# caofff/GL-ABC-MCMC

Hardware: NVIDIA B200
Metric: abc_mcmc_chain_steps_per_sec (higher is better)
Workload: dtype f32

## Files before the change

### gl-abc-mcmc_b200/csrc/philox.cuh

```cuda
#pragma once
#include <cstdint>
#include <cuda_runtime.h>

namespace glabc {

constexpr uint32_t kPhiloxM0 = 0xD2511F53u;
constexpr uint32_t kPhiloxM1 = 0xCD9E8D57u;
constexpr uint32_t kPhiloxW0 = 0x9E3779B9u;
constexpr uint32_t kPhiloxW1 = 0xBB67AE85u;

constexpr uint32_t kSlotStep = 1u;
constexpr uint32_t kSlotNormal = 2u;
constexpr uint32_t kSlotU64 = 0x80000000u;

struct RoundKeys {
    uint32_t k[10][2];
};

__host__ __device__ inline RoundKeys expand_key(uint2 key)
{
    RoundKeys rk;
    for (int r = 0; r < 10; ++r) {
        rk.k[r][0] = key.x + static_cast<uint32_t>(r) * kPhiloxW0;
        rk.k[r][1] = key.y + static_cast<uint32_t>(r) * kPhiloxW1;
    }
    return rk;
}

__device__ __forceinline__ uint4 philox4x32_10(uint4 c, const RoundKeys& rk)
{
#pragma unroll
    for (int r = 0; r < 10; ++r) {
        const uint64_t p0 = static_cast<uint64_t>(kPhiloxM0) * c.x;
        const uint64_t p1 = static_cast<uint64_t>(kPhiloxM1) * c.z;
        c = make_uint4(static_cast<uint32_t>(p1 >> 32) ^ c.y ^ rk.k[r][0], static_cast<uint32_t>(p1),
                       static_cast<uint32_t>(p0 >> 32) ^ c.w ^ rk.k[r][1], static_cast<uint32_t>(p0));
    }
    return c;
}

struct Stream {
    uint32_t chain_lo, chain_hi;
    __device__ __forceinline__ uint4 block(const RoundKeys& rk, uint32_t blk, uint32_t slot) const
    {
        return philox4x32_10(make_uint4(chain_lo, chain_hi, blk, slot), rk);
    }
};

__device__ __forceinline__ float u24(uint32_t w) { return __uint2float_rn(w >> 8) * 0x1p-24f; }

__device__ __forceinline__ float lg2_approx(float x)
{
    float r;
    asm("lg2.approx.ftz.f32 %0, %1;" : "=f"(r) : "f"(x));
    return r;
}

__device__ __forceinline__ float log_approx(float x) { return 0.69314718055994531f * lg2_approx(x); }

__device__ __forceinline__ void box_muller(uint32_t w0, uint32_t w1, float& n0, float& n1)
{
    const float u1 = fmaf(__uint2float_rn(w0 & 0xFFFFFF00u), 0x1p-32f, 0x1p-25f);
    const float r2 = -1.3862943611198906f * lg2_approx(u1);
    float r;
    asm("sqrt.approx.ftz.f32 %0, %1;" : "=f"(r) : "f"(r2));
    const float a = __uint2float_rn(w1 & 0xFFFFF000u) * (6.28318530717958647692f * 0x1p-32f);
    n0 = r * __cosf(a);
    n1 = r * __sinf(a);
}

__device__ __forceinline__ uint32_t step_block_ub(const uint4& w) { return __byte_perm(w.x, w.z, 0x0400); }
__device__ __forceinline__ uint32_t step_block_ua(const uint4& w) { return (w.y & 0xFFFu) | ((w.w << 12) & 0xFFF000u); }

}
```

### gl-abc-mcmc_b200/csrc/sampler_common.cuh

```cuda
#pragma once
#include <cstdint>
#include <cuda_runtime.h>

#include "../../include/glabc.h"
#include "model.cuh"
#include "philox.cuh"

namespace glabc {

struct RunParams {
    int32_t n_chains;
    uint32_t first_step;
    uint32_t last_step;
    uint32_t chain_lo0, chain_hi0;
    RoundKeys rk;
    float gf;
    uint32_t gf_thr_hi;
    int32_t gf_all_global;
    int32_t write_row0;
    int64_t trace_rows, trace_chains, trace_chain_off, trace_row_base;
    float* theta;
    float* y;
    float* aux;
    float* trace;
    float* stats;
    const float* tape32;
    const double* tape64;
    float* debug;
    float* tape_dump;
    double* tape64_dump;
    int32_t n_candidates;
    int32_t trace_layout;
    double* state64;
    const float* tape_grad0;
    float* tape_grad0_dump;
    double* debug64;
};

__device__ __forceinline__ Stream chain_stream(const RunParams& r, int32_t chain)
{
    const uint64_t gid = (static_cast<uint64_t>(r.chain_hi0) << 32 | r.chain_lo0) + static_cast<uint64_t>(chain);
    return Stream{static_cast<uint32_t>(gid), static_cast<uint32_t>(gid >> 32)};
}

template <int D>
struct VecOf { using type = float; };
template <> struct VecOf<2> { using type = float2; };
template <> struct VecOf<4> { using type = float4; };

template <int D>
__device__ __forceinline__ void store_row(float* dst, const float (&v)[D])
{
    if constexpr (D == 2) {
        *reinterpret_cast<float2*>(dst) = make_float2(v[0], v[1]);
    } else if constexpr (D == 4) {
        *reinterpret_cast<float4*>(dst) = make_float4(v[0], v[1], v[2], v[3]);
    } else {
#pragma unroll
        for (int k = 0; k < D; ++k) dst[k] = v[k];
    }
}

template <int D>
struct TimeMajorWriter {
    float* next;
    bool active;
    __device__ __forceinline__ TimeMajorWriter(const RunParams& r, int32_t chain, bool act, float*)
        : active(act)
    {
        const int64_t first_row = static_cast<int64_t>(r.first_step) - (r.write_row0 ? 1 : 0) - r.trace_row_base;
        next = r.trace + (first_row * r.trace_chains + r.trace_chain_off + chain) * D;
    }
    __device__ __forceinline__ void put(const RunParams& r, uint32_t, const float (&v)[D])
    {
        if (active) store_row<D>(next, v);
        next += r.trace_chains * D;
    }
    __device__ __forceinline__ void maybe_flush(const RunParams&, uint32_t) {}
    __device__ __forceinline__ void finish(const RunParams&) {}
    static constexpr int smem_floats_per_warp = 0;
};

template <int D>
struct ChainMajorWriter {
    static constexpr int kPitch = 33;
    static constexpr int kPlane = 32 * kPitch + (D > 1 ? 32 / D : 0);
    static constexpr int smem_floats_per_warp = D * kPlane;
    float* tile;
    float* out;
    int64_t chain_stride;
    uint32_t row0;
    int32_t count;
    int32_t lane;
    int32_t chains_in_warp;

    __device__ __forceinline__ ChainMajorWriter(const RunParams& r, int32_t, bool, float* smem_warp)
        : tile(smem_warp), chain_stride(r.trace_rows * D), row0(0), count(0), lane(threadIdx.x & 31)
    {
        const int32_t chain0 = blockIdx.x * blockDim.x + (threadIdx.x & ~31u);
        out = r.trace + (r.trace_chain_off + chain0) * chain_stride;
        chains_in_warp = min(32, r.n_chains - chain0);
    }

    __device__ __forceinline__ void put(const RunParams& r, uint32_t row, const float (&v)[D])
    {
        if (count == 0) row0 = row;
#pragma unroll
        for (int k = 0; k < D; ++k) tile[k * kPlane + count * kPitch + lane] = v[k];
        ++count;
    }

    __device__ __forceinline__ void maybe_flush(const RunParams& r, uint32_t row)
    {
        if (((row + 1u) & 31u) == 0u) flush(r);
    }

    __device__ __forceinline__ void flush(const RunParams& r)
    {
        __syncwarp();
        const int32_t n = count * D;
        const int64_t off = (static_cast<int64_t>(row0) - r.trace_row_base) * D;
        for (int32_t c = 0; c < chains_in_warp; ++c) {
            float* dst = out + c * chain_stride + off;
            for (int32_t e = lane; e < n; e += 32) {
                const int32_t s = e / D, k = e - s * D;
                dst[e] = tile[k * kPlane + s * kPitch + c];
            }
        }
        __syncwarp();
        count = 0;
    }

    __device__ __forceinline__ void finish(const RunParams& r)
    {
        if (count > 0) flush(r);
    }
};

template <int D>
struct ChainMajorVecWriter {
    using V = typename VecOf<D>::type;
    static constexpr int kPitch = 33;
    static constexpr int smem_floats_per_warp = 32 * kPitch * D;
    V* tile;
    V* out;
    int64_t chain_stride;
    uint32_t row0;
    int32_t count, lane, chains_in_warp;

    __device__ __forceinline__ ChainMajorVecWriter(const RunParams& r, int32_t, bool, float* smem_warp)
        : tile(reinterpret_cast<V*>(smem_warp)), chain_stride(r.trace_rows), row0(0), count(0), lane(threadIdx.x & 31)
    {
        const int32_t chain0 = blockIdx.x * blockDim.x + (threadIdx.x & ~31u);
        out = reinterpret_cast<V*>(r.trace) + (r.trace_chain_off + chain0) * chain_stride;
        chains_in_warp = min(32, r.n_chains - chain0);
    }

    __device__ __forceinline__ void put(const RunParams&, uint32_t row, const float (&v)[D])
    {
        if (count == 0) row0 = row;
        V x;
        if constexpr (D == 1) x = v[0];
        else if constexpr (D == 2) x = make_float2(v[0], v[1]);
        else x = make_float4(v[0], v[1], v[2], v[3]);
        tile[count * kPitch + lane] = x;
        ++count;
    }

    __device__ __forceinline__ void maybe_flush(const RunParams& r, uint32_t row)
    {
        if (((row + 1u) & 31u) == 0u) flush(r);
    }

    __device__ __forceinline__ void flush(const RunParams& r)
    {
        __syncwarp();
        V* dst = out + (static_cast<int64_t>(row0) - r.trace_row_base) + lane;
        const V* src = tile + lane * kPitch;
        if (count == 32 && chains_in_warp == 32) {
#pragma unroll 8
            for (int32_t c = 0; c < 32; ++c) dst[c * chain_stride] = src[c];
        } else {
            for (int32_t c = 0; c < chains_in_warp; ++c)
                if (lane < count) dst[c * chain_stride] = src[c];
        }
        __syncwarp();
        count = 0;
    }

    __device__ __forceinline__ void finish(const RunParams& r)
    {
        if (count > 0) flush(r);
    }
};

template <int D>
struct EventWriter {
    float* ev;
    uint32_t n;
    uint32_t cap;
    float last[D];
    bool active;
    static constexpr int smem_floats_per_warp = 0;
    __device__ __forceinline__ EventWriter(const RunParams& r, int32_t chain, bool act, float*)
        : ev(r.trace + (r.trace_chain_off + chain) * r.trace_rows * (1 + D)), n(1u), cap(static_cast<uint32_t>(r.trace_rows)), active(act)
    {
#pragma unroll
        for (int k = 0; k < D; ++k) last[k] = __int_as_float(0x7fc00000);
    }
    __device__ __forceinline__ void put(const RunParams&, uint32_t row, const float (&v)[D])
    {
        bool moved = false;
#pragma unroll
        for (int k = 0; k < D; ++k) moved |= !(v[k] == last[k]);
        if (moved) {
            if (active && n < cap) {
                float* e = ev + static_cast<int64_t>(n) * (1 + D);
                e[0] = __uint_as_float(row);
#pragma unroll
                for (int k = 0; k < D; ++k) e[1 + k] = v[k];
            }
            ++n;
#pragma unroll
            for (int k = 0; k < D; ++k) last[k] = v[k];
        }
    }
    __device__ __forceinline__ void maybe_flush(const RunParams&, uint32_t) {}
    __device__ __forceinline__ void finish(const RunParams&)
    {
        if (active) ev[0] = __uint_as_float(n - 1u);
    }
};

struct NoTraceWriter {
    __device__ __forceinline__ NoTraceWriter(const RunParams&, int32_t, bool, float*) {}
    template <int D>
    __device__ __forceinline__ void put(const RunParams&, uint32_t, const float (&)[D]) {}
    __device__ __forceinline__ void maybe_flush(const RunParams&, uint32_t) {}
    __device__ __forceinline__ void finish(const RunParams&) {}
    static constexpr int smem_floats_per_warp = 0;
};

template <int D, int LAYOUT> struct WriterFor;
template <int D> struct WriterFor<D, GLABC_TRACE_NONE> { using type = NoTraceWriter; };
template <int D> struct WriterFor<D, GLABC_TRACE_TIME_MAJOR> { using type = TimeMajorWriter<D>; };
template <int D> struct WriterFor<D, GLABC_TRACE_CHAIN_MAJOR> { using type = ChainMajorVecWriter<D>; };
template <> struct WriterFor<3, GLABC_TRACE_CHAIN_MAJOR> { using type = ChainMajorWriter<3>; };
template <int D> struct WriterFor<D, GLABC_TRACE_EVENTS> { using type = EventWriter<D>; };

template <int D>
struct ChainStats {
    static constexpr int kTri = D * (D + 1) / 2;
    uint32_t n_global, acc_local, acc_global;
    float f_global, f_acc, f_acc_global;
    float sum[D], sumsq[D], gram[kTri];

    __device__ __forceinline__ ChainStats()
        : n_global(0), acc_local(0), acc_global(0), f_global(0.0f), f_acc(0.0f), f_acc_global(0.0f)
    {
#pragma unroll
        for (int i = 0; i < D; ++i) sum[i] = sumsq[i] = 0.0f;
#pragma unroll
        for (int i = 0; i < kTri; ++i) gram[i] = 0.0f;
    }

    __device__ __forceinline__ void update(bool is_global, bool moved, const float (&theta_new)[D],
                                           const float (&theta_prev)[D])
    {
        n_global += is_global;
        acc_global += (moved && is_global);
        acc_local += (moved && !is_global);
        float dl[D];
#pragma unroll
        for (int i = 0; i < D; ++i) {
            sum[i] += theta_new[i];
            sumsq[i] = fmaf(theta_new[i], theta_new[i], sumsq[i]);
            dl[i] = theta_new[i] - theta_prev[i];
        }
        int t = 0;
#pragma unroll
        for (int i = 0; i < D; ++i)
#pragma unroll
            for (int j = i; j < D; ++j, ++t) gram[t] = fmaf(dl[i], dl[j], gram[t]);
    }

    __device__ __forceinline__ void update_masked(float glob, float moved, const float (&theta_new)[D],
                                                  const float (&theta_prev)[D])
    {
        f_global += glob;
        f_acc += moved;
        f_acc_global = fmaf(moved, glob, f_acc_global);
        float dl[D];
#pragma unroll
        for (int i = 0; i < D; ++i) {
            sum[i] += theta_new[i];
            sumsq[i] = fmaf(theta_new[i], theta_new[i], sumsq[i]);
            dl[i] = theta_new[i] - theta_prev[i];
        }
        int t = 0;
#pragma unroll
        for (int i = 0; i < D; ++i)
#pragma unroll
            for (int j = i; j < D; ++j, ++t) gram[t] = fmaf(dl[i], dl[j], gram[t]);
    }

    __device__ __forceinline__ void store(float* st, uint32_t n_steps) const
    {
        st[GLABC_STAT_STEPS] += static_cast<float>(n_steps);
        st[GLABC_STAT_GLOBAL_STEPS] += static_cast<float>(n_global) + f_global;
        st[GLABC_STAT_ACC_LOCAL] += static_cast<float>(acc_local) + (f_acc - f_acc_global);
        st[GLABC_STAT_ACC_GLOBAL] += static_cast<float>(acc_global) + f_acc_global;
#pragma unroll
        for (int i = 0; i < D; ++i) {
            st[GLABC_STAT_SUM + i] += sum[i];
            st[GLABC_STAT_SUM + D + i] += sumsq[i];
        }
#pragma unroll
        for (int i = 0; i < kTri; ++i) st[GLABC_STAT_SUM + 2 * D + i] += gram[i];
    }
};

}
```

### gl-abc-mcmc_b200/csrc/step_global.cuh

```cuda
#pragma once
#include "launch.cuh"
#include "sampler_common.cuh"

namespace glabc {

struct GlobalConsts {
    ModelConsts model;
    GaussConsts lp;
    GaussConsts gp;
};

template <int D>
struct StepInputs {
    bool is_global;
    float keep;
    float glob;
    float cand[D];
    float noise[D];
    float lq_p;
    float log_w;
    float raw[2 * D + 2];
};

template <int D, bool STRICT, bool KEEP_RAW>
__device__ __forceinline__ StepInputs<D> make_inputs(const GlobalConsts& K, bool is_global, float u_b, float u_a,
                                                    const float (&eps_p)[D], const float (&eps_s)[D])
{
    StepInputs<D> in;
    in.is_global = is_global;
    in.keep = is_global ? 0.0f : 1.0f;
    in.glob = 1.0f - in.keep;
    if constexpr (STRICT) {
        float th_g[D], th_l[D];
        in.lq_p = gauss_forward<D, true>(K.gp, eps_p, th_g);
        (void)gauss_forward<D, true>(K.lp, eps_p, th_l);
#pragma unroll
        for (int k = 0; k < D; ++k) {
            in.cand[k] = is_global ? th_g[k] : th_l[k];
            in.noise[k] = __fadd_rn(K.model.noise_loc[k], __fmul_rn(K.model.noise_scale[k], eps_s[k]));
        }
        in.log_w = logf(u_a);
    } else {
        float q = 0.0f;
#pragma unroll
        for (int k = 0; k < D; ++k) {
            const float cg = fmaf(K.gp.scale[k], eps_p[k], K.gp.loc[k]);
            const float cl = fmaf(K.lp.scale[k], eps_p[k], K.lp.loc[k]);
            in.cand[k] = is_global ? cg : cl;
            in.noise[k] = fmaf(K.model.noise_scale[k], eps_s[k], K.model.noise_loc[k]);
            q = fmaf(eps_p[k], eps_p[k], q);
        }
        in.lq_p = fmaf(-0.5f, q, K.gp.c_fast);
        in.log_w = fmaf(in.glob, in.lq_p, log_approx(u_a));
    }
    if constexpr (KEEP_RAW) {
        in.raw[0] = u_b;
#pragma unroll
        for (int k = 0; k < D; ++k) {
            in.raw[1 + k] = eps_p[k];
            in.raw[1 + D + k] = eps_s[k];
        }
        in.raw[1 + 2 * D] = u_a;
    }
    return in;
}

template <int D, bool STRICT>
__device__ __forceinline__ StepInputs<D> inputs_from_tape(const GlobalConsts& K, const RunParams& r,
                                                         uint32_t step_in_launch, int32_t chain)
{
    constexpr int kSlots = GLABC_TAPE_GLOBAL_SLOTS(D, D);
    const float* t = r.tape32 + (static_cast<int64_t>(step_in_launch) * kSlots) * r.n_chains + chain;
    float eps_p[D], eps_s[D];
    const float u_b = __ldg(t);
#pragma unroll
    for (int k = 0; k < D; ++k) eps_p[k] = __ldg(t + static_cast<int64_t>(1 + k) * r.n_chains);
#pragma unroll
    for (int k = 0; k < D; ++k) eps_s[k] = __ldg(t + static_cast<int64_t>(1 + D + k) * r.n_chains);
    const float u_a = __ldg(t + static_cast<int64_t>(1 + 2 * D) * r.n_chains);
    return make_inputs<D, STRICT, false>(K, u_b < r.gf, u_b, u_a, eps_p, eps_s);
}

template <int D, bool STRICT, bool KEEP_RAW>
__device__ __forceinline__ StepInputs<D> inputs_native(const GlobalConsts& K, const RunParams& r, const RoundKeys& rk,
                                                      const Stream& s, uint32_t step)
{
    constexpr int kGroups = (2 * D + 3) / 4;
    float z[kGroups * 4];
    const uint4 w0 = s.block(rk, step, kSlotStep);
    box_muller(w0.x, w0.y, z[0], z[1]);
    box_muller(w0.z, w0.w, z[2], z[3]);
#pragma unroll
    for (int g = 1; g < kGroups; ++g) {
        const uint4 w = s.block(rk, step, kSlotNormal + g - 1);
        box_muller(w.x, w.y, z[4 * g + 0], z[4 * g + 1]);
        box_muller(w.z, w.w, z[4 * g + 2], z[4 * g + 3]);
    }
    float eps_p[D], eps_s[D];
#pragma unroll
    for (int k = 0; k < D; ++k) {
        eps_p[k] = z[k];
        eps_s[k] = z[D + k];
    }
    const uint32_t ub = step_block_ub(w0);
    const bool is_global = (ub < r.gf_thr_hi) || r.gf_all_global;
    const float u_a = __uint2float_rn(step_block_ua(w0)) * 0x1p-24f;
    return make_inputs<D, STRICT, KEEP_RAW>(K, is_global, KEEP_RAW ? __uint2float_rn(ub >> 16) * 0x1p-16f : 0.0f, u_a, eps_p, eps_s);
}

template <int D>
struct ChainState {
    float theta[D], y[D];
    float prior, kern;
};

struct StepRecord {
    float prior_p, kern_p, log_acc;
    bool accept;
};

template <int D, int FAMILY, bool STRICT>
__device__ __forceinline__ StepRecord advance(const GlobalConsts& K, ChainState<D>& st, ChainStats<D>& stats,
                                              const StepInputs<D>& in)
{
    float theta_p[D], y_p[D];
    if constexpr (!STRICT) {
        float qp = 0.0f, sk = 0.0f, qo = 0.0f;
#pragma unroll
        for (int k = 0; k < D; ++k) {
            theta_p[k] = fmaf(in.keep, st.theta[k], in.cand[k]);
            y_p[k] = (FAMILY == GLABC_MODEL_ABS_NORMAL ? fabsf(theta_p[k]) : theta_p[k]) + in.noise[k];
            const float dy = y_p[k] - K.model.y_obs[k];
            sk = fmaf(dy, dy, sk);
            const float rp = fmaf(theta_p[k], K.model.prior.inv_scale[k], K.model.prior.nloc_inv[k]);
            qp = fmaf(rp, rp, qp);
            const float ro = fmaf(st.theta[k], K.gp.inv_scale[k], K.gp.nloc_inv[k]);
            qo = fmaf(ro, ro, qo);
        }
        const float tgt_p = fmaf(K.model.kern_fast_m, sk, fmaf(-0.5f, qp, K.model.prior.c_fast + K.model.kern_fast_c));
        const float lq_old = fmaf(-0.5f, qo, K.gp.c_fast);
        const float rhs = fmaf(in.glob, lq_old, tgt_p - st.prior);
        const bool accept = in.log_w < rhs;
        float prev[D];
#pragma unroll
        for (int k = 0; k < D; ++k) {
            prev[k] = st.theta[k];
            st.theta[k] = accept ? theta_p[k] : st.theta[k];
            st.y[k] = accept ? y_p[k] : st.y[k];
        }
        st.prior = accept ? tgt_p : st.prior;
        stats.update_masked(in.glob, accept ? 1.0f : 0.0f, st.theta, prev);
        return StepRecord{fmaf(-0.5f, qp, K.model.prior.c_fast), fmaf(K.model.kern_fast_m, sk, K.model.kern_fast_c),
                          fmaf(-in.glob, in.lq_p, rhs), accept};
    }
#pragma unroll
    for (int k = 0; k < D; ++k) {
        theta_p[k] = in.is_global ? in.cand[k] : __fadd_rn(in.cand[k], st.theta[k]);
        const float mean = FAMILY == GLABC_MODEL_ABS_NORMAL ? fabsf(theta_p[k]) : theta_p[k];
        y_p[k] = __fadd_rn(mean, in.noise[k]);
    }
    const float prior_p = model_prior<D, STRICT>(K.model, theta_p);
    const float kern_p = model_log_kernel<D, STRICT>(K.model, y_p);
    const float lq_old = gauss_log_prob<D, STRICT>(K.gp, st.theta);
    float log_acc;
    if constexpr (STRICT) {
        const float base = __fadd_rn(prior_p, kern_p);
        const float g = __fsub_rn(__fsub_rn(__fsub_rn(__fadd_rn(base, lq_old), in.lq_p), st.prior), st.kern);
        const float l = __fsub_rn(__fsub_rn(base, st.prior), st.kern);
        log_acc = in.is_global ? g : l;
    } else {
        const float corr = in.is_global ? lq_old - in.lq_p : 0.0f;
        log_acc = (prior_p + kern_p) + (corr - (st.prior + st.kern));
    }
    const bool accept = in.log_w < log_acc;

    float prev[D];
#pragma unroll
    for (int k = 0; k < D; ++k) {
        prev[k] = st.theta[k];
        st.theta[k] = accept ? theta_p[k] : st.theta[k];
        st.y[k] = accept ? y_p[k] : st.y[k];
    }
    st.prior = accept ? prior_p : st.prior;
    st.kern = accept ? kern_p : st.kern;
    stats.update(in.is_global, accept, st.theta, prev);
    return StepRecord{prior_p, kern_p, log_acc, accept};
}

template <int D, int FAMILY, bool STRICT, bool REPLAY, int LAYOUT, bool DUMP>
__global__ void __launch_bounds__(256) k_global_mcmc(const __grid_constant__ GlobalConsts K,
                                                     const __grid_constant__ RunParams R)
{
    using Writer = typename WriterFor<D, LAYOUT>::type;
    extern __shared__ float smem[];
    const int32_t chain = blockIdx.x * blockDim.x + threadIdx.x;
    const bool active = chain < R.n_chains;
    const int32_t cidx = active ? chain : R.n_chains - 1;

    ChainState<D> st;
#pragma unroll
    for (int k = 0; k < D; ++k) {
        st.theta[k] = R.theta[static_cast<int64_t>(cidx) * D + k];
        st.y[k] = R.y[static_cast<int64_t>(cidx) * D + k];
    }
    st.prior = model_prior<D, STRICT>(K.model, st.theta);
    st.kern = model_log_kernel<D, STRICT>(K.model, st.y);
    if constexpr (!STRICT) st.prior += st.kern;

    Writer writer(R, cidx, active, smem + (threadIdx.x >> 5) * Writer::smem_floats_per_warp);
    if (R.write_row0) {
        writer.put(R, R.first_step - 1u, st.theta);
        writer.maybe_flush(R, R.first_step - 1u);
    }
    ChainStats<D> stats;

    if constexpr (REPLAY) {
        for (uint32_t i = R.first_step; i <= R.last_step && R.last_step >= R.first_step; ++i) {
            const StepInputs<D> in = inputs_from_tape<D, STRICT>(K, R, i - R.first_step, cidx);
            const StepRecord rec = advance<D, FAMILY, STRICT>(K, st, stats, in);
            writer.put(R, i, st.theta);
            writer.maybe_flush(R, i);
            if (R.debug != nullptr && active) {
                float* g = R.debug + static_cast<int64_t>(i - R.first_step) * GLABC_DEBUG_SLOTS * R.n_chains + chain;
                g[0] = static_cast<float>(static_cast<int>(in.is_global) | (static_cast<int>(rec.accept) << 1));
                g[static_cast<int64_t>(1) * R.n_chains] = rec.prior_p;
                g[static_cast<int64_t>(2) * R.n_chains] = rec.kern_p;
                g[static_cast<int64_t>(3) * R.n_chains] = rec.log_acc;
            }
        }
    } else {
        const Stream stream = chain_stream(R, cidx);
        auto dump = [&](uint32_t i, const StepInputs<D>& in) {
            if constexpr (DUMP) {
                if (R.tape_dump != nullptr && active) {
                    constexpr int kSlots = GLABC_TAPE_GLOBAL_SLOTS(D, D);
                    float* t = R.tape_dump + static_cast<int64_t>(i - R.first_step) * kSlots * R.n_chains + chain;
#pragma unroll
                    for (int k = 0; k < kSlots; ++k) t[static_cast<int64_t>(k) * R.n_chains] = in.raw[k];
                }
            }
        };
        auto single = [&](uint32_t i) {
            const StepInputs<D> in = inputs_native<D, STRICT, DUMP>(K, R, R.rk, stream, i);
            advance<D, FAMILY, STRICT>(K, st, stats, in);
            writer.put(R, i, st.theta);
            writer.maybe_flush(R, i);
            dump(i, in);
        };
        auto prepare4 = [&](uint32_t i, StepInputs<D> (&b)[4]) {
#pragma unroll
            for (int k = 0; k < 4; ++k) b[k] = inputs_native<D, STRICT, DUMP>(K, R, R.rk, stream, i + k);
        };
        auto advance4 = [&](uint32_t i, const StepInputs<D> (&b)[4]) {
#pragma unroll
            for (int k = 0; k < 4; ++k) {
                advance<D, FAMILY, STRICT>(K, st, stats, b[k]);
                writer.put(R, i + k, st.theta);
                dump(i + k, b[k]);
            }
            writer.maybe_flush(R, i + 3u);
        };

        if (R.last_step >= R.first_step) {
            uint32_t i = R.first_step;
            while (i <= R.last_step && (i & 3u)) single(i++);
            if (i + 3u <= R.last_step) {
                StepInputs<D> a[4], b[4];
                prepare4(i, a);
                while (i + 11u <= R.last_step) {
                    prepare4(i + 4u, b);
                    advance4(i, a);
                    prepare4(i + 8u, a);
                    advance4(i + 4u, b);
                    i += 8u;
                }
                if (i + 7u <= R.last_step) {
                    prepare4(i + 4u, b);
                    advance4(i, a);
                    advance4(i + 4u, b);
                    i += 8u;
                } else {
                    advance4(i, a);
                    i += 4u;
                }
            }
            while (i <= R.last_step) single(i++);
        }
    }
    writer.finish(R);

    if (active) {
#pragma unroll
        for (int k = 0; k < D; ++k) {
            R.theta[static_cast<int64_t>(chain) * D + k] = st.theta[k];
            R.y[static_cast<int64_t>(chain) * D + k] = st.y[k];
        }
        if (R.stats != nullptr)
            stats.store(R.stats + static_cast<int64_t>(chain) * GLABC_NSTATS(D), R.last_step + 1u - R.first_step);
    }
}

template <int D, int FAMILY, bool STRICT, bool REPLAY, int LAYOUT, bool DUMP>
static cudaError_t launch_one(const GlobalConsts& K, const RunParams& R, int block, cudaStream_t st)
{
    using Writer = typename WriterFor<D, LAYOUT>::type;
    const int grid = (R.n_chains + block - 1) / block;
    const size_t smem = sizeof(float) * Writer::smem_floats_per_warp * (block / 32);
    auto kern = k_global_mcmc<D, FAMILY, STRICT, REPLAY, LAYOUT, DUMP>;
    if (smem > 48 * 1024) {
        cudaError_t e = cudaFuncSetAttribute(kern, cudaFuncAttributeMaxDynamicSharedMemorySize, static_cast<int>(smem));
        if (e != cudaSuccess) return e;
    }
    kern<<<grid, block, smem, st>>>(K, R);
    return cudaGetLastError();
}

template <int D, int FAMILY, bool STRICT>
static cudaError_t launch_mode(const GlobalConsts& K, const RunParams& R, bool replay, int layout, int block, cudaStream_t st)
{
    if (replay) {
        switch (layout) {
        case GLABC_TRACE_NONE: return launch_one<D, FAMILY, STRICT, true, GLABC_TRACE_NONE, false>(K, R, block, st);
        case GLABC_TRACE_TIME_MAJOR: return launch_one<D, FAMILY, STRICT, true, GLABC_TRACE_TIME_MAJOR, false>(K, R, block, st);
        case GLABC_TRACE_CHAIN_MAJOR: return launch_one<D, FAMILY, STRICT, true, GLABC_TRACE_CHAIN_MAJOR, false>(K, R, block, st);
        }
        return cudaErrorInvalidValue;
    }
    if (R.tape_dump != nullptr) {
        if (layout != GLABC_TRACE_TIME_MAJOR) return cudaErrorInvalidValue;
        return launch_one<D, FAMILY, STRICT, false, GLABC_TRACE_TIME_MAJOR, true>(K, R, block, st);
    }
    switch (layout) {
    case GLABC_TRACE_NONE: return launch_one<D, FAMILY, STRICT, false, GLABC_TRACE_NONE, false>(K, R, block, st);
    case GLABC_TRACE_TIME_MAJOR: return launch_one<D, FAMILY, STRICT, false, GLABC_TRACE_TIME_MAJOR, false>(K, R, block, st);
    case GLABC_TRACE_CHAIN_MAJOR: return launch_one<D, FAMILY, STRICT, false, GLABC_TRACE_CHAIN_MAJOR, false>(K, R, block, st);
    case GLABC_TRACE_EVENTS: return launch_one<D, FAMILY, STRICT, false, GLABC_TRACE_EVENTS, false>(K, R, block, st);
    }
    return cudaErrorInvalidValue;
}

template <int D>
cudaError_t launch_global_mcmc_dim(const ModelConsts& model, const GaussConsts& lp, const GaussConsts& gp,
                                   const RunParams& R, bool strict, bool replay, int layout, int block, cudaStream_t st)
{
    GlobalConsts K{model, lp, gp};
    return with_family(model.family, [&](auto f) {
        return strict ? launch_mode<D, f, true>(K, R, replay, layout, block, st)
                      : launch_mode<D, f, false>(K, R, replay, layout, block, st);
    });
}

}
```

Measured before the change: 152.4 billion.

## Hoist chain-invariant Philox rounds and add tiled chain-major trace writer

Precomputes the parts of the first two Philox rounds of the per-step random block that depend only on the chain counter, so each step runs fewer multiply rounds when the chain high word is uniform. Adds a shared-memory tiled chain-major trace writer for D=1,2,4 that buffers 32 steps per lane and writes them out as coalesced vector stores, and realigns the unrolled loop to 8-step groups so slot indices are compile-time constants. The costs are extra shared memory per warp, which may lower occupancy, and a runtime branch that compiles two loop bodies. A profiling script is also added.

```diff
diff --git a/gl-abc-mcmc_b200/csrc/philox.cuh b/gl-abc-mcmc_b200/csrc/philox.cuh
--- a/gl-abc-mcmc_b200/csrc/philox.cuh
+++ b/gl-abc-mcmc_b200/csrc/philox.cuh
@@ -27,10 +27,11 @@
     return rk;
 }
 
-__device__ __forceinline__ uint4 philox4x32_10(uint4 c, const RoundKeys& rk)
+template <int R0>
+__device__ __forceinline__ uint4 philox_rounds(uint4 c, const RoundKeys& rk)
 {
 #pragma unroll
-    for (int r = 0; r < 10; ++r) {
+    for (int r = R0; r < 10; ++r) {
         const uint64_t p0 = static_cast<uint64_t>(kPhiloxM0) * c.x;
         const uint64_t p1 = static_cast<uint64_t>(kPhiloxM1) * c.z;
         c = make_uint4(static_cast<uint32_t>(p1 >> 32) ^ c.y ^ rk.k[r][0], static_cast<uint32_t>(p1),
@@ -39,12 +40,45 @@
     return c;
 }
 
+__device__ __forceinline__ uint4 philox4x32_10(uint4 c, const RoundKeys& rk) { return philox_rounds<0>(c, rk); }
+
 struct Stream {
     uint32_t chain_lo, chain_hi;
     __device__ __forceinline__ uint4 block(const RoundKeys& rk, uint32_t blk, uint32_t slot) const
     {
         return philox4x32_10(make_uint4(chain_lo, chain_hi, blk, slot), rk);
     }
+};
+
+struct StepBlockHoisted {
+    const uint32_t& chain_hi;
+    uint32_t w1;
+    uint32_t x2, y2;
+
+    __device__ __forceinline__ StepBlockHoisted(uint32_t chain_lo, const uint32_t& hi, const RoundKeys& rk) : chain_hi(hi)
+    {
+        const uint64_t p0 = static_cast<uint64_t>(kPhiloxM0) * chain_lo;
+        w1 = static_cast<uint32_t>(p0);
+        const uint32_t z1 = static_cast<uint32_t>(p0 >> 32) ^ kSlotStep ^ rk.k[0][1];
+        const uint64_t p1 = static_cast<uint64_t>(kPhiloxM1) * z1;
+        x2 = static_cast<uint32_t>(p1 >> 32) ^ rk.k[1][0];
+        y2 = static_cast<uint32_t>(p1);
+    }
+
+    __device__ __forceinline__ uint4 operator()(const RoundKeys& rk, uint32_t step) const
+    {
+        const uint64_t p1 = static_cast<uint64_t>(kPhiloxM1) * step;
+        const uint32_t x1 = static_cast<uint32_t>(p1 >> 32) ^ chain_hi ^ rk.k[0][0];
+        const uint64_t p0 = static_cast<uint64_t>(kPhiloxM0) * x1;
+        const uint4 c = make_uint4(x2 ^ static_cast<uint32_t>(p1), y2, static_cast<uint32_t>(p0 >> 32) ^ w1 ^ rk.k[1][1],
+                                   static_cast<uint32_t>(p0));
+        return philox_rounds<2>(c, rk);
+    }
+};
+
+struct StepBlockRef {
+    Stream s;
+    __device__ __forceinline__ uint4 operator()(const RoundKeys& rk, uint32_t step) const { return s.block(rk, step, kSlotStep); }
 };
 
 __device__ __forceinline__ float u24(uint32_t w) { return __uint2float_rn(w >> 8) * 0x1p-24f; }
diff --git a/gl-abc-mcmc_b200/csrc/sampler_common.cuh b/gl-abc-mcmc_b200/csrc/sampler_common.cuh
--- a/gl-abc-mcmc_b200/csrc/sampler_common.cuh
+++ b/gl-abc-mcmc_b200/csrc/sampler_common.cuh
@@ -19,6 +19,7 @@
     int32_t gf_all_global;
     int32_t write_row0;
     int64_t trace_rows, trace_chains, trace_chain_off, trace_row_base;
+    int32_t chain_hi_uniform;
     float* theta;
     float* y;
     float* aux;
@@ -195,6 +196,70 @@
 };
 
 template <int D>
+struct ChainMajorTileWriter {
+    static_assert(D == 1 || D == 2 || D == 4, "vector rows only");
+    using V = typename VecOf<D>::type;
+    static constexpr int kPitch = 33;
+    static constexpr int smem_floats_per_warp = 32 * kPitch * D;
+    V* slots;
+
+    __device__ __forceinline__ ChainMajorTileWriter(const RunParams&, int32_t, bool, float* smem_warp)
+        : slots(reinterpret_cast<V*>(smem_warp) + (threadIdx.x & 31) * kPitch) {}
+
+    static __device__ __forceinline__ V vec(const float (&v)[D])
+    {
+        if constexpr (D == 1) return v[0];
+        else if constexpr (D == 2) return make_float2(v[0], v[1]);
+        else return make_float4(v[0], v[1], v[2], v[3]);
+    }
+
+    __device__ __forceinline__ void put(const RunParams&, uint32_t row, const float (&v)[D]) { slots[row & 31u] = vec(v); }
+
+    template <int S>
+    __device__ __forceinline__ void put_static(const RunParams&, uint32_t i8, const float (&v)[D])
+    {
+        slots[(i8 & 31u) + S] = vec(v);
+    }
+
+    __device__ __forceinline__ void maybe_flush(const RunParams& r, uint32_t row)
+    {
+        if (((row + 1u) & 31u) == 0u) flush(r, row);
+    }
+
+    __device__ __forceinline__ void flush(const RunParams& r, uint32_t last)
+    {
+        __syncwarp();
+        const uint32_t lane = threadIdx.x & 31u;
+        const uint32_t row0 = last & ~31u;
+        const uint32_t first = r.first_step - (r.write_row0 ? 1u : 0u);
+        const int32_t chain0 = blockIdx.x * blockDim.x + (threadIdx.x & ~31u);
+        const int32_t n = min(32, r.n_chains - chain0);
+        const V* tile = slots - lane * kPitch;
+        V* dst = reinterpret_cast<V*>(r.trace) + (r.trace_chain_off + chain0) * r.trace_rows + (static_cast<int64_t>(row0) - r.trace_row_base) + lane;
+        const int64_t stride_bytes = r.trace_rows * static_cast<int64_t>(sizeof(V));
+        if (first <= row0 && (last & 31u) == 31u && n == 32 && (stride_bytes >> 32) == 0) {
+            const uint32_t sb = static_cast<uint32_t>(stride_bytes);
+#pragma unroll
+            for (uint32_t c = 0; c < 32; ++c)
+                *reinterpret_cast<V*>(reinterpret_cast<char*>(dst) + static_cast<uint64_t>(sb) * c) = tile[c * kPitch + lane];
+        } else {
+            const uint32_t s0 = first > row0 ? first - row0 : 0u, s1 = last & 31u;
+            if (lane >= s0 && lane <= s1) {
+#pragma unroll 1
+                for (int32_t c = 0; c < n; ++c) dst[c * r.trace_rows] = tile[c * kPitch + lane];
+            }
+        }
+        __syncwarp();
+    }
+
+    __device__ __forceinline__ void finish(const RunParams& r)
+    {
+        const uint32_t first = r.first_step - (r.write_row0 ? 1u : 0u);
+        if (r.last_step >= first && ((r.last_step + 1u) & 31u) != 0u) flush(r, r.last_step);
+    }
+};
+
+template <int D>
 struct EventWriter {
     float* ev;
     uint32_t n;
diff --git a/gl-abc-mcmc_b200/csrc/step_global.cuh b/gl-abc-mcmc_b200/csrc/step_global.cuh
--- a/gl-abc-mcmc_b200/csrc/step_global.cuh
+++ b/gl-abc-mcmc_b200/csrc/step_global.cuh
@@ -81,13 +81,13 @@
     return make_inputs<D, STRICT, false>(K, u_b < r.gf, u_b, u_a, eps_p, eps_s);
 }
 
-template <int D, bool STRICT, bool KEEP_RAW>
+template <int D, bool STRICT, bool KEEP_RAW, class StepBlock>
 __device__ __forceinline__ StepInputs<D> inputs_native(const GlobalConsts& K, const RunParams& r, const RoundKeys& rk,
-                                                      const Stream& s, uint32_t step)
+                                                      const Stream& s, const StepBlock& step_block, uint32_t step)
 {
     constexpr int kGroups = (2 * D + 3) / 4;
     float z[kGroups * 4];
-    const uint4 w0 = s.block(rk, step, kSlotStep);
+    const uint4 w0 = step_block(rk, step);
     box_muller(w0.x, w0.y, z[0], z[1]);
     box_muller(w0.z, w0.w, z[2], z[3]);
 #pragma unroll
@@ -187,11 +187,19 @@
     return StepRecord{prior_p, kern_p, log_acc, accept};
 }
 
+template <int D, int LAYOUT> struct GlobalWriterFor { using type = typename WriterFor<D, LAYOUT>::type; };
+template <> struct GlobalWriterFor<1, GLABC_TRACE_CHAIN_MAJOR> { using type = ChainMajorTileWriter<1>; };
+template <> struct GlobalWriterFor<2, GLABC_TRACE_CHAIN_MAJOR> { using type = ChainMajorTileWriter<2>; };
+template <> struct GlobalWriterFor<4, GLABC_TRACE_CHAIN_MAJOR> { using type = ChainMajorTileWriter<4>; };
+
+template <class W> struct HasStaticSlots { static constexpr bool value = false; };
+template <int D> struct HasStaticSlots<ChainMajorTileWriter<D>> { static constexpr bool value = true; };
+
 template <int D, int FAMILY, bool STRICT, bool REPLAY, int LAYOUT, bool DUMP>
 __global__ void __launch_bounds__(256) k_global_mcmc(const __grid_constant__ GlobalConsts K,
                                                      const __grid_constant__ RunParams R)
 {
-    using Writer = typename WriterFor<D, LAYOUT>::type;
+    using Writer = typename GlobalWriterFor<D, LAYOUT>::type;
     extern __shared__ float smem[];
     const int32_t chain = blockIdx.x * blockDim.x + threadIdx.x;
     const bool active = chain < R.n_chains;
@@ -240,52 +248,65 @@
                 }
             }
         };
-        auto single = [&](uint32_t i) {
-            const StepInputs<D> in = inputs_native<D, STRICT, DUMP>(K, R, R.rk, stream, i);
-            advance<D, FAMILY, STRICT>(K, st, stats, in);
-            writer.put(R, i, st.theta);
-            writer.maybe_flush(R, i);
-            dump(i, in);
+        auto native = [&](const auto& step_block) {
+            auto single = [&](uint32_t i) {
+                const StepInputs<D> in = inputs_native<D, STRICT, DUMP>(K, R, R.rk, stream, step_block, i);
+                advance<D, FAMILY, STRICT>(K, st, stats, in);
+                writer.put(R, i, st.theta);
+                writer.maybe_flush(R, i);
+                dump(i, in);
+            };
+            auto prepare4 = [&](uint32_t i, StepInputs<D> (&b)[4]) {
+#pragma unroll
+                for (int k = 0; k < 4; ++k) b[k] = inputs_native<D, STRICT, DUMP>(K, R, R.rk, stream, step_block, i + k);
+            };
+            auto step_at = [&](uint32_t i8, const StepInputs<D>& in, auto s) {
+                constexpr int S = decltype(s)::value;
+                advance<D, FAMILY, STRICT>(K, st, stats, in);
+                if constexpr (HasStaticSlots<Writer>::value) writer.template put_static<S>(R, i8, st.theta);
+                else writer.put(R, i8 + S, st.theta);
+                dump(i8 + S, in);
+            };
+            auto advance4 = [&](uint32_t i8, const StepInputs<D> (&b)[4], auto h) {
+                constexpr int H = decltype(h)::value;
+                step_at(i8, b[0], std::integral_constant<int, H + 0>{});
+                step_at(i8, b[1], std::integral_constant<int, H + 1>{});
+                step_at(i8, b[2], std::integral_constant<int, H + 2>{});
+                step_at(i8, b[3], std::integral_constant<int, H + 3>{});
+            };
+            constexpr std::integral_constant<int, 0> lo{};
+            constexpr std::integral_constant<int, 4> hi{};
+
+            if (R.last_step >= R.first_step) {
+                uint32_t i = R.first_step;
+                while (i <= R.last_step && (i & 7u)) single(i++);
+                if (i + 3u <= R.last_step) {
+                    StepInputs<D> a[4], b[4];
+                    prepare4(i, a);
+                    while (i + 11u <= R.last_step) {
+                        prepare4(i + 4u, b);
+                        advance4(i, a, lo);
+                        prepare4(i + 8u, a);
+                        advance4(i, b, hi);
+                        writer.maybe_flush(R, i + 7u);
+                        i += 8u;
+                    }
+                    if (i + 7u <= R.last_step) {
+                        prepare4(i + 4u, b);
+                        advance4(i, a, lo);
+                        advance4(i, b, hi);
+                        writer.maybe_flush(R, i + 7u);
+                        i += 8u;
+                    } else {
+                        advance4(i, a, lo);
+                        i += 4u;
+                    }
+                }
+                while (i <= R.last_step) single(i++);
+            }
         };
-        auto prepare4 = [&](uint32_t i, StepInputs<D> (&b)[4]) {
-#pragma unroll
-            for (int k = 0; k < 4; ++k) b[k] = inputs_native<D, STRICT, DUMP>(K, R, R.rk, stream, i + k);
-        };
-        auto advance4 = [&](uint32_t i, const StepInputs<D> (&b)[4]) {
-#pragma unroll
-            for (int k = 0; k < 4; ++k) {
-                advance<D, FAMILY, STRICT>(K, st, stats, b[k]);
-                writer.put(R, i + k, st.theta);
-                dump(i + k, b[k]);
-            }
-            writer.maybe_flush(R, i + 3u);
-        };
-
-        if (R.last_step >= R.first_step) {
-            uint32_t i = R.first_step;
-            while (i <= R.last_step && (i & 3u)) single(i++);
-            if (i + 3u <= R.last_step) {
-                StepInputs<D> a[4], b[4];
-                prepare4(i, a);
-                while (i + 11u <= R.last_step) {
-                    prepare4(i + 4u, b);
-                    advance4(i, a);
-                    prepare4(i + 8u, a);
-                    advance4(i + 4u, b);
-                    i += 8u;
-                }
-                if (i + 7u <= R.last_step) {
-                    prepare4(i + 4u, b);
-                    advance4(i, a);
-                    advance4(i + 4u, b);
-                    i += 8u;
-                } else {
-                    advance4(i, a);
-                    i += 4u;
-                }
-            }
-            while (i <= R.last_step) single(i++);
-        }
+        if (R.chain_hi_uniform) native(StepBlockHoisted(stream.chain_lo, R.chain_hi0, R.rk));
+        else native(StepBlockRef{stream});
     }
     writer.finish(R);
 
@@ -303,7 +324,7 @@
 template <int D, int FAMILY, bool STRICT, bool REPLAY, int LAYOUT, bool DUMP>
 static cudaError_t launch_one(const GlobalConsts& K, const RunParams& R, int block, cudaStream_t st)
 {
-    using Writer = typename WriterFor<D, LAYOUT>::type;
+    using Writer = typename GlobalWriterFor<D, LAYOUT>::type;
     const int grid = (R.n_chains + block - 1) / block;
     const size_t smem = sizeof(float) * Writer::smem_floats_per_warp * (block / 32);
     auto kern = k_global_mcmc<D, FAMILY, STRICT, REPLAY, LAYOUT, DUMP>;
@@ -344,9 +365,11 @@
                                    const RunParams& R, bool strict, bool replay, int layout, int block, cudaStream_t st)
 {
     GlobalConsts K{model, lp, gp};
+    RunParams P = R;
+    P.chain_hi_uniform = static_cast<uint64_t>(R.chain_lo0) + static_cast<uint64_t>(R.n_chains) <= (uint64_t{1} << 32);
     return with_family(model.family, [&](auto f) {
-        return strict ? launch_mode<D, f, true>(K, R, replay, layout, block, st)
-                      : launch_mode<D, f, false>(K, R, replay, layout, block, st);
+        return strict ? launch_mode<D, f, true>(K, P, replay, layout, block, st)
+                      : launch_mode<D, f, false>(K, P, replay, layout, block, st);
     });
 }
 
diff --git a/profiles/micro/k1_trace_writer.py b/profiles/micro/k1_trace_writer.py
--- /dev/null
+++ b/profiles/micro/k1_trace_writer.py
@@ -0,0 +1,134 @@
+import argparse
+import json
+import os
+import subprocess
+import sys
+
+ROOT = os.path.dirname(os.path.dirname(os.path.dirname(os.path.abspath(__file__))))
+LAYOUTS = ("none", "time", "chain")
+
+
+def smi(query):
+    p = subprocess.run(["nvidia-smi", "--id=0", f"--query-gpu={query}", "--format=csv,noheader"], capture_output=True, text=True)
+    return p.stdout.strip() or p.stderr.strip()
+
+
+def child(layouts, warmup, timed, chains, iters):
+    import torch
+    sys.path.insert(0, ROOT)
+    import glabc_b200 as g
+    from glabc_b200 import _abi as abi
+    from glabc_b200.engine import get_engine
+
+    torch.cuda.set_device(0)
+    eng = get_engine()
+    eng.bind_model(g.Mixture_set(0.05))
+    eng.bind_proposal(abi.SLOT_LOCAL, g.DiagGaussian(2, torch.zeros(1, 2), torch.log(torch.tensor([0.35, 0.35]))))
+    eng.bind_proposal(abi.SLOT_GLOBAL, g.DiagGaussian(2, torch.zeros(2), torch.zeros(2)))
+    C, T, d = chains, iters, 2
+    gen = torch.Generator(device="cuda").manual_seed(1234)
+    theta0 = torch.zeros(C, d, device="cuda")
+    y0 = torch.randn(C, d, device="cuda", generator=gen) * 0.22360679507255554
+    theta, y = theta0.clone(), y0.clone()
+    stats = torch.zeros(C, abi.nstats(d), device="cuda")
+    out = {}
+    for name in layouts:
+        layout = {"chain": abi.TRACE_CHAIN_MAJOR, "time": abi.TRACE_TIME_MAJOR, "none": abi.TRACE_NONE}[name]
+        trace = None
+        if layout != abi.TRACE_NONE:
+            trace = torch.empty((C, T, d) if layout == abi.TRACE_CHAIN_MAJOR else (T, C, d), device="cuda")
+        ms = []
+        for s in range(warmup + timed):
+            theta.copy_(theta0)
+            y.copy_(y0)
+            e0, e1 = torch.cuda.Event(enable_timing=True), torch.cuda.Event(enable_timing=True)
+            e0.record()
+            eng.run("global", theta=theta, y=y, n_steps=T - 1, gf=0.5, seed=s, trace_layout=layout, trace=trace,
+                    trace_rows=T, stats=stats)
+            e1.record()
+            torch.cuda.synchronize()
+            if s >= warmup:
+                ms.append(e0.elapsed_time(e1))
+        del trace
+        torch.cuda.empty_cache()
+        mean = sum(ms) / len(ms)
+        out[name] = {"mean_ms": mean, "min_ms": min(ms), "max_ms": max(ms),
+                     "chain_steps_per_sec": C * (T - 1) / (mean * 1e-3)}
+    print(json.dumps(out))
+
+
+def sass_loop(lib, layout):
+    import collections
+    import re
+    name = f"_ZN5glabc13k_global_mcmcILi2ELi1ELb0ELb0ELi{layout}ELb0EEEvNS_12GlobalConstsENS_9RunParamsE"
+    p = subprocess.run(["cuobjdump", "-sass", "-fun", name, lib], capture_output=True, text=True, check=True)
+    ins = [(int(m.group(1), 16), m.group(2).strip()) for m in
+           (re.match(r"\s*/\*([0-9a-f]{4,})\*/\s+(.*?);", l) for l in p.stdout.splitlines()) if m]
+    at = {a: k for k, (a, _) in enumerate(ins)}
+    op = lambda t: re.sub(r"^@!?U?P\w+\s+", "", t).split()[0]
+    branches = []
+    for k, (a, t) in enumerate(ins):
+        m = re.search(r"BRA\S*\s+.*?0x([0-9a-f]+)\s*$", t)
+        if m and int(m.group(1), 16) in at:
+            branches.append((k, at[int(m.group(1), 16)], t.startswith("@")))
+    loops = sorted(((k - j, j, k) for k, j, _ in branches if j < k), reverse=True)
+    results = []
+    for _, s, e in loops[:2]:
+        flush = set()
+        for k, j, cond in branches:
+            if cond and s <= k < j <= e and any(op(t).startswith("STG") for _, t in ins[k + 1:j]):
+                flush.update(range(k + 1, j))
+        ops = collections.Counter(op(t) for _, t in ins[s:e + 1])
+        body = e + 1 - s - len(flush)
+        lane_imad_wide = sum(1 for k in range(s, e + 1) if k not in flush and re.search(r"(^|\s)IMAD\.WIDE\.U32\s", ins[k][1]))
+        results.append({"loop_instructions": e + 1 - s, "flush_instructions": len(flush), "body_per_step": body / 8,
+                        "lane_imad_wide_per_step": lane_imad_wide / 8,
+                        "const_reloads_per_step": sum(v for o, v in ops.items() if o.startswith(("LDC", "LDCU"))) / 8,
+                        "uniform_imad_wide": ops.get("UIMAD.WIDE.U32", 0)})
+    return results
+
+
+def main():
+    p = argparse.ArgumentParser()
+    p.add_argument("--sass", metavar="LIB", help="print the static main-loop counts of LIB and exit (no GPU)")
+    p.add_argument("--lib", action="append", default=[], help="name=path of a libglabc build (repeatable)")
+    p.add_argument("--rounds", type=int, default=3)
+    p.add_argument("--layouts", default=",".join(LAYOUTS))
+    p.add_argument("--warmup", type=int, default=3)
+    p.add_argument("--timed", type=int, default=20)
+    p.add_argument("--chains", type=int, default=65536)
+    p.add_argument("--iters", type=int, default=10000)
+    p.add_argument("--child", action="store_true")
+    a = p.parse_args()
+    layouts = a.layouts.split(",")
+    if a.sass:
+        for name, layout in (("none", 0), ("time", 1), ("chain", 2)):
+            print(name, json.dumps(sass_loop(a.sass, layout)))
+        return
+    if a.child:
+        child(layouts, a.warmup, a.timed, a.chains, a.iters)
+        return
+    libs = [tuple(s.split("=", 1)) for s in a.lib] or [("tree", os.path.join(ROOT, "gl-abc-mcmc_b200", "csrc", "libglabc.so"))]
+    print("card:", smi("name,power.limit,clocks.sm,clocks.max.sm"), flush=True)
+    res = {name: {l: [] for l in layouts} for name, _ in libs}
+    for r in range(a.rounds):
+        for name, path in libs:
+            env = dict(os.environ, GLABC_LIB=os.path.abspath(path))
+            cmd = [sys.executable, os.path.abspath(__file__), "--child", "--layouts", a.layouts, "--warmup", str(a.warmup),
+                   "--timed", str(a.timed), "--chains", str(a.chains), "--iters", str(a.iters)]
+            p = subprocess.run(cmd, env=env, capture_output=True, text=True)
+            if p.returncode != 0:
+                sys.exit(f"{name} failed:\n{p.stderr[-3000:]}")
+            got = json.loads(p.stdout.strip().splitlines()[-1])
+            for l in layouts:
+                res[name][l].append(got[l]["mean_ms"])
+            print(f"round {r} {name:>6}: " + "  ".join(f"{l} {got[l]['mean_ms']:.4f} ms [{got[l]['min_ms']:.4f}, {got[l]['max_ms']:.4f}]"
+                                                      for l in layouts) + f"   sm clock now {smi('clocks.sm')}", flush=True)
+    print("mean over rounds (spread = max - min of the round means):")
+    for name, _ in libs:
+        print(f"{name:>6}: " + "  ".join(f"{l} {sum(v) / len(v):.4f} ms (spread {max(v) - min(v):.4f})" for l, v in res[name].items()))
+    print(json.dumps(res))
+
+
+if __name__ == "__main__":
+    main()
```

Result: faster. 154.0 billion (median of 6 runs) (+1.0%).

## Tile chain-major trace writes per 32 steps and use 16-byte flush stores

Applied to the files above, without the earlier changes.

For the chain-major trace layout, the step loop now runs in 32-step tiles. Each step writes into a fixed shared-memory slot, and the tile is flushed once at the end of the tile, which removes the per-step count bookkeeping and the per-4-step flush check. For D=2, when the trace pointer and row counts are 16-byte compatible, the flush writes two float2 rows per lane as float4 stores, with a padded pitch of 34. This trades some added code paths and a larger shared-memory pitch for fewer, wider global stores and less loop control overhead.

```diff
diff --git a/gl-abc-mcmc_b200/csrc/sampler_common.cuh b/gl-abc-mcmc_b200/csrc/sampler_common.cuh
--- a/gl-abc-mcmc_b200/csrc/sampler_common.cuh
+++ b/gl-abc-mcmc_b200/csrc/sampler_common.cuh
@@ -18,6 +18,7 @@
     uint32_t gf_thr_hi;
     int32_t gf_all_global;
     int32_t write_row0;
+    int32_t trace_runs_16b;
     int64_t trace_rows, trace_chains, trace_chain_off, trace_row_base;
     float* theta;
     float* y;
@@ -135,35 +136,52 @@
     {
         if (count > 0) flush(r);
     }
-};
-
-template <int D>
+
+    __device__ __forceinline__ void put_slot(uint32_t slot, const float (&v)[D])
+    {
+#pragma unroll
+        for (int k = 0; k < D; ++k) tile[k * kPlane + slot * kPitch + lane] = v[k];
+    }
+    __device__ __forceinline__ void flush_tile(const RunParams& r, uint32_t first_row)
+    {
+        row0 = first_row;
+        count = 32;
+        flush(r);
+    }
+};
+
+template <int D, bool WIDE = false>
 struct ChainMajorVecWriter {
+    static_assert(!WIDE || D == 2, "the 16-byte flush moves two float2 rows per lane");
     using V = typename VecOf<D>::type;
-    static constexpr int kPitch = 33;
+    static constexpr int kPitch = WIDE ? 34 : 33;
     static constexpr int smem_floats_per_warp = 32 * kPitch * D;
-    V* tile;
+    V* line;
     V* out;
     int64_t chain_stride;
     uint32_t row0;
     int32_t count, lane, chains_in_warp;
 
     __device__ __forceinline__ ChainMajorVecWriter(const RunParams& r, int32_t, bool, float* smem_warp)
-        : tile(reinterpret_cast<V*>(smem_warp)), chain_stride(r.trace_rows), row0(0), count(0), lane(threadIdx.x & 31)
+        : chain_stride(r.trace_rows), row0(0), count(0), lane(threadIdx.x & 31)
     {
         const int32_t chain0 = blockIdx.x * blockDim.x + (threadIdx.x & ~31u);
-        out = reinterpret_cast<V*>(r.trace) + (r.trace_chain_off + chain0) * chain_stride;
+        line = reinterpret_cast<V*>(smem_warp) + lane * kPitch;
+        out = reinterpret_cast<V*>(r.trace) + ((r.trace_chain_off + chain0) * chain_stride - r.trace_row_base);
         chains_in_warp = min(32, r.n_chains - chain0);
     }
 
+    static __device__ __forceinline__ V pack(const float (&v)[D])
+    {
+        if constexpr (D == 1) return v[0];
+        else if constexpr (D == 2) return make_float2(v[0], v[1]);
+        else return make_float4(v[0], v[1], v[2], v[3]);
+    }
+
     __device__ __forceinline__ void put(const RunParams&, uint32_t row, const float (&v)[D])
     {
         if (count == 0) row0 = row;
-        V x;
-        if constexpr (D == 1) x = v[0];
-        else if constexpr (D == 2) x = make_float2(v[0], v[1]);
-        else x = make_float4(v[0], v[1], v[2], v[3]);
-        tile[count * kPitch + lane] = x;
+        line[count] = pack(v);
         ++count;
     }
 
@@ -174,25 +192,48 @@
 
     __device__ __forceinline__ void flush(const RunParams& r)
     {
+        flush_rows(r, row0, count);
+        count = 0;
+    }
+
+    __device__ __forceinline__ void finish(const RunParams& r)
+    {
+        if (count > 0) flush(r);
+    }
+
+    __device__ __forceinline__ void put_slot(uint32_t slot, const float (&v)[D]) { line[slot] = pack(v); }
+    __device__ __forceinline__ void flush_tile(const RunParams& r, uint32_t first_row) { flush_rows(r, first_row, 32); }
+
+    __device__ __forceinline__ void flush_rows(const RunParams& r, uint32_t first_row, int32_t n)
+    {
         __syncwarp();
-        V* dst = out + (static_cast<int64_t>(row0) - r.trace_row_base) + lane;
-        const V* src = tile + lane * kPitch;
-        if (count == 32 && chains_in_warp == 32) {
+        const V* tile = line - lane * kPitch;
+        if (n == 32 && chains_in_warp == 32) {
+            if (WIDE && r.trace_runs_16b) {
+                const int32_t h = lane >> 4, j = 2 * (lane & 15);
+                const V* src = tile + h * kPitch + j;
+                V* dst = out + h * chain_stride + first_row + j;
+#pragma unroll
+                for (int32_t c = 0; c < 32; c += 2)
+                    *reinterpret_cast<float4*>(dst + c * chain_stride) = *reinterpret_cast<const float4*>(src + c * kPitch);
+            } else {
+                V* dst = out + first_row + lane;
 #pragma unroll 8
-            for (int32_t c = 0; c < 32; ++c) dst[c * chain_stride] = src[c];
+                for (int32_t c = 0; c < 32; ++c) dst[c * chain_stride] = tile[c * kPitch + lane];
+            }
         } else {
+            V* dst = out + first_row + lane;
             for (int32_t c = 0; c < chains_in_warp; ++c)
-                if (lane < count) dst[c * chain_stride] = src[c];
+                if (lane < n) dst[c * chain_stride] = tile[c * kPitch + lane];
         }
         __syncwarp();
-        count = 0;
-    }
-
-    __device__ __forceinline__ void finish(const RunParams& r)
-    {
-        if (count > 0) flush(r);
-    }
-};
+    }
+};
+
+inline bool chain_major_runs_16b(const RunParams& r)
+{
+    return (reinterpret_cast<uintptr_t>(r.trace) & 15u) == 0 && (r.trace_rows & 1) == 0 && (r.trace_row_base & 1) == 0;
+}
 
 template <int D>
 struct EventWriter {
@@ -241,12 +282,12 @@
     static constexpr int smem_floats_per_warp = 0;
 };
 
-template <int D, int LAYOUT> struct WriterFor;
-template <int D> struct WriterFor<D, GLABC_TRACE_NONE> { using type = NoTraceWriter; };
-template <int D> struct WriterFor<D, GLABC_TRACE_TIME_MAJOR> { using type = TimeMajorWriter<D>; };
-template <int D> struct WriterFor<D, GLABC_TRACE_CHAIN_MAJOR> { using type = ChainMajorVecWriter<D>; };
-template <> struct WriterFor<3, GLABC_TRACE_CHAIN_MAJOR> { using type = ChainMajorWriter<3>; };
-template <int D> struct WriterFor<D, GLABC_TRACE_EVENTS> { using type = EventWriter<D>; };
+template <int D, int LAYOUT, bool WIDE = false> struct WriterFor;
+template <int D, bool W> struct WriterFor<D, GLABC_TRACE_NONE, W> { using type = NoTraceWriter; };
+template <int D, bool W> struct WriterFor<D, GLABC_TRACE_TIME_MAJOR, W> { using type = TimeMajorWriter<D>; };
+template <int D, bool W> struct WriterFor<D, GLABC_TRACE_CHAIN_MAJOR, W> { using type = ChainMajorVecWriter<D, W && D == 2>; };
+template <bool W> struct WriterFor<3, GLABC_TRACE_CHAIN_MAJOR, W> { using type = ChainMajorWriter<3>; };
+template <int D, bool W> struct WriterFor<D, GLABC_TRACE_EVENTS, W> { using type = EventWriter<D>; };
 
 template <int D>
 struct ChainStats {
diff --git a/gl-abc-mcmc_b200/csrc/step_global.cuh b/gl-abc-mcmc_b200/csrc/step_global.cuh
--- a/gl-abc-mcmc_b200/csrc/step_global.cuh
+++ b/gl-abc-mcmc_b200/csrc/step_global.cuh
@@ -191,7 +191,7 @@
 __global__ void __launch_bounds__(256) k_global_mcmc(const __grid_constant__ GlobalConsts K,
                                                      const __grid_constant__ RunParams R)
 {
-    using Writer = typename WriterFor<D, LAYOUT>::type;
+    using Writer = typename WriterFor<D, LAYOUT, true>::type;
     extern __shared__ float smem[];
     const int32_t chain = blockIdx.x * blockDim.x + threadIdx.x;
     const bool active = chain < R.n_chains;
@@ -251,38 +251,35 @@
 #pragma unroll
             for (int k = 0; k < 4; ++k) b[k] = inputs_native<D, STRICT, DUMP>(K, R, R.rk, stream, i + k);
         };
-        auto advance4 = [&](uint32_t i, const StepInputs<D> (&b)[4]) {
+        constexpr bool kTiled = LAYOUT == GLABC_TRACE_CHAIN_MAJOR;
+        constexpr uint32_t kTile = kTiled ? 32u : 8u;
+        auto advance4 = [&](uint32_t i, uint32_t slot, const StepInputs<D> (&b)[4]) {
 #pragma unroll
             for (int k = 0; k < 4; ++k) {
                 advance<D, FAMILY, STRICT>(K, st, stats, b[k]);
-                writer.put(R, i + k, st.theta);
+                if constexpr (kTiled) writer.put_slot(slot + k, st.theta);
+                else writer.put(R, i + k, st.theta);
                 dump(i + k, b[k]);
             }
-            writer.maybe_flush(R, i + 3u);
         };
 
         if (R.last_step >= R.first_step) {
             uint32_t i = R.first_step;
-            while (i <= R.last_step && (i & 3u)) single(i++);
-            if (i + 3u <= R.last_step) {
+            while (i <= R.last_step && (i % kTile)) single(i++);
+            if (i + (kTile - 1u) <= R.last_step) {
                 StepInputs<D> a[4], b[4];
                 prepare4(i, a);
-                while (i + 11u <= R.last_step) {
-                    prepare4(i + 4u, b);
-                    advance4(i, a);
-                    prepare4(i + 8u, a);
-                    advance4(i + 4u, b);
-                    i += 8u;
-                }
-                if (i + 7u <= R.last_step) {
-                    prepare4(i + 4u, b);
-                    advance4(i, a);
-                    advance4(i + 4u, b);
-                    i += 8u;
-                } else {
-                    advance4(i, a);
-                    i += 4u;
-                }
+                do {
+#pragma unroll 1
+                    for (uint32_t s = 0; s < kTile; s += 8u) {
+                        prepare4(i + s + 4u, b);
+                        advance4(i + s, s, a);
+                        prepare4(i + s + 8u, a);
+                        advance4(i + s + 4u, s + 4u, b);
+                    }
+                    if constexpr (kTiled) writer.flush_tile(R, i);
+                    i += kTile;
+                } while (i + (kTile - 1u) <= R.last_step);
             }
             while (i <= R.last_step) single(i++);
         }
@@ -303,7 +300,7 @@
 template <int D, int FAMILY, bool STRICT, bool REPLAY, int LAYOUT, bool DUMP>
 static cudaError_t launch_one(const GlobalConsts& K, const RunParams& R, int block, cudaStream_t st)
 {
-    using Writer = typename WriterFor<D, LAYOUT>::type;
+    using Writer = typename WriterFor<D, LAYOUT, true>::type;
     const int grid = (R.n_chains + block - 1) / block;
     const size_t smem = sizeof(float) * Writer::smem_floats_per_warp * (block / 32);
     auto kern = k_global_mcmc<D, FAMILY, STRICT, REPLAY, LAYOUT, DUMP>;
@@ -311,7 +308,9 @@
         cudaError_t e = cudaFuncSetAttribute(kern, cudaFuncAttributeMaxDynamicSharedMemorySize, static_cast<int>(smem));
         if (e != cudaSuccess) return e;
     }
-    kern<<<grid, block, smem, st>>>(K, R);
+    RunParams P = R;
+    P.trace_runs_16b = LAYOUT == GLABC_TRACE_CHAIN_MAJOR && D == 2 && chain_major_runs_16b(R);
+    kern<<<grid, block, smem, st>>>(K, P);
     return cudaGetLastError();
 }
 
diff --git a/profiles/micro/k1_sass_count.py b/profiles/micro/k1_sass_count.py
--- /dev/null
+++ b/profiles/micro/k1_sass_count.py
@@ -0,0 +1,114 @@
+import collections
+import importlib
+import os
+import re
+import subprocess
+import sys
+import tempfile
+
+ROOT = os.path.dirname(os.path.dirname(os.path.dirname(os.path.abspath(__file__))))
+sys.path.insert(0, ROOT)
+build = importlib.import_module("gl-abc-mcmc_b200.build")
+LAYOUTS = {"TRACE_NONE": 0, "TRACE_TIME_MAJOR": 1, "TRACE_CHAIN_MAJOR": 2}
+
+
+def mangled(layout):
+    return f"_ZN5glabc13k_global_mcmcILi2ELi1ELb0ELb0ELi{layout}ELb0EEEvNS_12GlobalConstsENS_9RunParamsE"
+
+
+def opcode(text):
+    t = text.split()
+    return (t[1] if t[0].startswith("@") else t[0]).split(".")[0]
+
+
+def parse(sass):
+    ins = []
+    for line in sass.splitlines():
+        m = re.match(r"\s*/\*([0-9a-f]{4,})\*/\s+(.*?)\s*;", line)
+        if m:
+            ins.append((int(m.group(1), 16), m.group(2).strip()))
+    return ins
+
+
+def branch_target(text):
+    m = re.search(r"\bBRA(?:\.\w+)*\s+(?:!?U?P\w+,\s*)?(0x[0-9a-f]+)", text)
+    return int(m.group(1), 16) if m else None
+
+
+def loops(ins):
+    where = {a: i for i, (a, _) in enumerate(ins)}
+    out = []
+    for i, (a, t) in enumerate(ins):
+        tgt = branch_target(t)
+        if tgt is not None and tgt < a and tgt in where:
+            out.append((where[tgt], i))
+    return out
+
+
+def outside_bssy(body):
+    depth, n = 0, []
+    for t in body:
+        op = opcode(t)
+        if op == "BSSY":
+            depth += 1
+        elif op == "BSYNC":
+            depth -= 1
+        elif depth == 0:
+            n.append(t)
+    return n
+
+
+def fall_through_path(ins, lo, hi, skip):
+    where = {a: i for i, (a, _) in enumerate(ins)}
+    i, n = lo, 0
+    while i < hi:
+        if skip[0] <= i <= skip[1]:
+            i = skip[1] + 1
+            continue
+        a, t = ins[i]
+        n += 1
+        tgt = branch_target(t)
+        if tgt is not None and re.match(r"BRA(\.U)?\s+0x", t):
+            i = where[tgt]
+        else:
+            i += 1
+    return n
+
+
+def count(ins):
+    ls = loops(ins)
+    mufu = lambda lo, hi: sum(opcode(t) == "MUFU" for _, t in ins[lo:hi + 1])
+    best = max(mufu(lo, hi) for lo, hi in ls)
+    step = min((l for l in ls if mufu(*l) == best), key=lambda l: l[1] - l[0])
+    body = [t for _, t in ins[step[0]:step[1] + 1]]
+    steady = len(outside_bssy(body)) / 8
+    enclosing = [l for l in ls if l[0] <= step[0] and l[1] > step[1]]
+    flushed = steady
+    if enclosing:
+        lo, hi = min(enclosing, key=lambda l: l[1] - l[0])
+        flushed = (4 * len(body) + fall_through_path(ins, lo, hi, step) + 1) / 32
+    ops = collections.Counter(opcode(t) for t in body)
+    return steady, flushed, {k: ops[k] for k in ("LDC", "LDCU", "S2R")}
+
+
+def main():
+    src = os.path.join(build.CSRC, "step_global_d2.cu")
+    flags = [f for f in build.NVCC_FLAGS if f not in ("-Xcompiler", "-fPIC", "-fvisibility=hidden")]
+    cuobjdump = os.path.join(os.path.dirname(build._nvcc()), "cuobjdump")
+    with tempfile.TemporaryDirectory() as tmp:
+        cubin = os.path.join(tmp, "d2.cubin")
+        p = subprocess.run([build._nvcc(), *flags, "-cubin", "-o", cubin, src], capture_output=True, text=True, check=True)
+        ptxas = p.stderr + p.stdout
+        print(f"{'layout':<20}{'steady':>8}{'flushed':>9}{'LDC':>5}{'LDCU':>6}{'S2R':>5}{'regs':>6}{'spill st/ld':>13}")
+        for name, lay in LAYOUTS.items():
+            fn = mangled(lay)
+            sass = subprocess.run([cuobjdump, "-sass", "-fun", fn, cubin], capture_output=True, text=True, check=True).stdout
+            steady, flushed, ops = count(parse(sass))
+            m = re.search(re.escape(fn) + r"\s*\n\s*(\d+) bytes stack frame, (\d+) bytes spill stores, (\d+) bytes spill loads"
+                          r"[\s\S]*?Used (\d+) registers", ptxas)
+            print(f"{name:<20}{steady:>8.2f}{flushed:>9.2f}{ops['LDC']:>5}{ops['LDCU']:>6}{ops['S2R']:>5}{m.group(4):>6}"
+                  f"{m.group(2) + '/' + m.group(3):>13}")
+
+
+if __name__ == "__main__":
+    main()
```

After: 152.2 billion before, 163.3 billion after (median of 6 runs). 7.3% higher.
